# ml4ai/iqlpref

Measured on AMD Instinct MI355X. Metric: iql_grad_steps_per_sec, higher is better.
Workload: dtype bf16; 1 GPU; IQL antmaze-medium-diverse-v2 shapes (S=29 A=8 H=256), 1M-transition device replay, batch 256, one seed per GPU; batch=256, buffer_rows=1000000, graph_unroll=0, graph_launches_per_block=0, eager_steps_per_block=1390

## Files before the change

### iqlpref_amd/csrc/api.hip

```cpp
#include <hip/hip_runtime.h>

#include <algorithm>
#include <cmath>
#include <cstdarg>
#include <cstdio>
#include <cstdlib>
#include <cstring>
#include <new>
#include <vector>

#include "../../include/iqlhip.h"
#include "common.h"
#include "errors.h"
#include "host_plan.h"
#include "iql_deep.h"
#include "iql_step.h"
#include "launchers.h"
#include "step_math.h"

using namespace iqlhip;

static thread_local char g_err[512] = "";
int iqlhip::fail(int code, const char *fmt, ...) {
  va_list ap;
// ... 482 lines not shown
      N.toff_w[k] = N.has_target ? N.off_w[k] : -1;
      N.toff_b[k] = N.has_target ? N.off_b[k] : -1;
    }
  }
  for (int n = 0; n < NT; ++n) {
    const TrainNet &N = D.net[n];
    std::vector<UpdItem> half[2];
    auto put = [&](int layer, int o0, int i0) {
      UpdItem it;
      memset(&it, 0, sizeof(it));
      it.net = n, it.layer = layer, it.o0 = o0, it.i0 = i0;
      it.Odim = (layer == 2) ? N.out_dim : H;
      it.Idim = (layer == 0) ? N.in_dim : H;
      it.Opad = (layer == 2) ? N.out_pad : H;
      it.Kw = (layer == 0) ? N.k1pad : H;
      it.has_target = N.has_target;
      it.group = n == D.net_v ? 1 : (n == D.net_a ? 2 : 0);
      it.off_w = N.off_w[layer], it.off_b = N.off_b[layer], it.toff_w = N.toff_w[layer], it.toff_b = N.toff_b[layer];
      half[(layer == 2 && it.Opad <= 64) ? ((i0 / 32) & 1) : (o0 >= it.Opad / 2 ? 1 : 0)].push_back(it);
    };
    for (int o0 = 0; o0 < H; o0 += 64)
      for (int i0 = 0; i0 < H; i0 += 32) put(1, o0, i0);
    for (int o0 = 0; o0 < H; o0 += strip_rows()) put(0, o0, 0);
    for (int o0 = 0; o0 < N.out_pad; o0 += 64)
      for (int i0 = 0; i0 < H; i0 += 32) put(2, o0, i0);
    u->n_half0[n] = (int)half[0].size();
    u->net_items[n] = half[0];
    u->net_items[n].insert(u->net_items[n].end(), half[1].begin(), half[1].end());
  }
  std::vector<UpdItem> items;
  {
    std::vector<UpdItem> per_xcd[8];
    deal_items(u, 0, 1, per_xcd);
    items = flatten_table(per_xcd, 0, nullptr, (size_t)(B + 15) / 16);
  }
  auto blocks = [&](WorkspacePlan p) {
    for (int n = 0; n < NT; ++n) {
      TrainNet &N = D.net[n];
      N.wc[0] = p.take<char>((size_t)H * N.k1pad * es);
      N.wc[1] = p.take<char>((size_t)H * H * es);
      N.wc[2] = p.take<char>((size_t)N.out_pad * H * es);
      if (N.has_target) {
        N.tc[0] = p.take<char>((size_t)H * N.k1pad * es);
        N.tc[1] = p.take<char>((size_t)H * H * es);
        N.tc[2] = p.take<char>((size_t)N.out_pad * H * es);
      }
      N.w2ct = p.take<char>((size_t)H * H * es);
      N.w3t = p.take<char>((size_t)H * N.out_pad * es);
    }
    D.xT = p.take<char>((size_t)2 * D.xrows * D.BP * es);
    D.rd = p.take<float>((size_t)B * 2);
    D.actf = p.take<float>((size_t)B * A);
    D.hT = p.take<char>((size_t)NT * 2 * H * D.BP * es);
    D.dz1T = p.take<char>((size_t)NT * H * D.BP * es);
    D.dz2T = p.take<char>((size_t)NT * H * D.BP * es);
    D.dz3T = p.take<char>((size_t)NT * D.opmax * D.BP * es);
    D.outs = p.take<float>((size_t)layer2_parts(H) * B * D.OUTW);
    D.lossp = p.take<float>((size_t)NT * (B / 16));
    D.lsp = p.take<float>((size_t)(B / 16) * A);
    D.ls_snap = p.take<float>((size_t)A);
    t->batch_rows = p.take<float>((size_t)B * stride);
    D.stage_rows = p.take<float>((size_t)B * stride);
    u->own.args = p.take<DevArgs>(1);
    u->own.ctr = p.take<DevCtr>(1);
    u->own.desc = p.take<TrainerDesc>(1);
    u->own.items = p.take<UpdItem>(items.size());
    return p.end();
  };
  const size_t total = blocks(WorkspacePlan());
  if (hipMalloc(&u->ws, total) != hipSuccess)
    return fail(IQLHIP_ERR_NOMEM, "hipMalloc of %zu workspace bytes failed", total);
  if (hipMemset(u->ws, 0, total) != hipSuccess) return fail(IQLHIP_ERR_HIP, "hipMemset failed");
  blocks(WorkspacePlan(u->ws));
  u->own.n_items = (int)items.size();
  u->cur = u->own;

  for (int n = 0; n < NT; ++n)
    for (auto &it : u->net_items[n]) item_pointers(it, D, es);
  for (auto &it : items) item_pointers(it, D, es);
  if (hipMemcpy(u->own.items, items.data(), items.size() * sizeof(UpdItem), hipMemcpyHostToDevice) != hipSuccess)
    return fail(IQLHIP_ERR_HIP, "hipMemcpy of the work items failed");

  const std::vector<EvalSpec> order = eval_order(sh, D.next_off);
  for (int f = 0; f < (int)order.size(); ++f) {
    const auto [net, target, in_off, out_col, slot] = order[f];
    FwdNet &F = D.fwd[f];
    const TrainNet &N = D.net[net];
    F.w1c = target ? N.tc[0] : N.wc[0];
    F.w2c = target ? N.tc[1] : N.wc[1];
    F.w3c = target ? N.tc[2] : N.wc[2];
    const float *base = target ? ar->target : ar->params;
    F.b1 = base + N.off_b[0], F.b2 = base + N.off_b[1], F.b3 = base + N.off_b[2];
    F.in_off = in_off, F.in_dim = N.in_dim, F.k1pad = N.k1pad;
// ... 694 lines not shown
```

### iqlpref_amd/csrc/common.h

```cpp
#pragma once
#include <hip/hip_runtime.h>
#include <stdint.h>

namespace iqlhip {

typedef __attribute__((ext_vector_type(4))) float f32x4;
typedef __attribute__((ext_vector_type(8))) __bf16 bf16x8;

constexpr int WAVE = 64;

__device__ __forceinline__ uint16_t f2bf(float x) {
  return __builtin_bit_cast(uint16_t, (__bf16)x);
}
__device__ __forceinline__ float bf2f(uint16_t h) {
  return __builtin_bit_cast(float, (uint32_t)h << 16);
}
__device__ __forceinline__ float rbf(float x) { return bf2f(f2bf(x)); }

#define IQL_AS1 __attribute__((address_space(1)))
template <class T>
__device__ __forceinline__ T ldg(const T *p) {
  return *(const T IQL_AS1 *)p;
}
template <class T>
// ... 100 lines not shown
  return v;
}

__host__ __device__ inline int round_up(int x, int m) { return (x + m - 1) / m * m; }

template <class P>
__host__ __device__ inline size_t fidx(int f, int k, int nk) {
  return ((((size_t)(f >> 4) * nk + k / P::KM) * 64) + ((k % P::KM) / P::EPV) * 16 + (f & 15)) * P::EPV +
         (k % P::EPV);
}
template <class P>
__host__ __device__ inline size_t frag_off(int ft, int ks, int nk, int lane) {
  return (((size_t)ft * nk + ks) * 64 + lane) * P::EPV;
}

struct Philox4 {
  uint32_t x, y, z, w;
};
__device__ __forceinline__ Philox4 philox4x32_10(uint32_t c0, uint32_t c1, uint32_t c2,
                                                 uint32_t c3, uint32_t k0, uint32_t k1) {
#pragma unroll
  for (int i = 0; i < 10; ++i) {
    const uint32_t hi0 = __umulhi(0xD2511F53u, c0), lo0 = 0xD2511F53u * c0;
    const uint32_t hi1 = __umulhi(0xCD9E8D57u, c2), lo1 = 0xCD9E8D57u * c2;
    c0 = hi1 ^ c1 ^ k0;
    c1 = lo1;
    c2 = hi0 ^ c3 ^ k1;
    c3 = lo0;
    k0 += 0x9E3779B9u;
    k1 += 0xBB67AE85u;
  }
  return Philox4{c0, c1, c2, c3};
}
constexpr uint32_t STREAM_INDEX = 0, STREAM_DROPOUT1 = 1, STREAM_DROPOUT2 = 2, STREAM_MLP_DROPOUT = 3;

__device__ __forceinline__ int64_t philox_index(uint64_t seed, uint64_t step, uint32_t row,
                                                uint64_t n_rows) {
  const Philox4 r = philox4x32_10(row, (uint32_t)step, (uint32_t)(step >> 32), STREAM_INDEX,
                                  (uint32_t)seed, (uint32_t)(seed >> 32));
  return (int64_t)((uint64_t)r.x % n_rows);
}

}
```

### iqlpref_amd/csrc/iql_step.h

```cpp
#pragma once
#include <hip/hip_runtime.h>
#include <stdint.h>

namespace iqlhip {

constexpr int MAX_CRITICS = 8;
constexpr int MAX_TRAIN = MAX_CRITICS + 2;
constexpr int MAX_FWD = 2 * MAX_CRITICS + 3;

struct FwdNet {
  const void *w1c, *w2c, *w3c;
  const float *b1, *b2, *b3;
  int32_t in_off;
  int32_t in_dim, k1pad;
  int32_t out_dim, out_pad;
  int32_t out_col;
  int32_t train_slot;
  int32_t tanh_out;
  int32_t dropout;
  int32_t stage;
};

struct TrainNet {
  int64_t off_w[3], off_b[3];
// ... 4 lines not shown
  void *tc[3];
  int32_t in_dim, k1pad, out_dim, out_pad;
  int32_t has_target;
};

struct TrainerDesc {
  int32_t S, A, H, B, BP, OUTW, k1max;
  int32_t E, ntrain, nfwd, net_v, net_a;
  int32_t out_v, out_qt, out_nv, out_mean;
  int32_t stage_stride, next_off;
  int32_t opmax, xrows;
  int32_t deterministic, has_dropout;
  int32_t prefetch;
  int32_t polyak_convex;
  float two_over_B, inv_E;
  float discount, tau, beta, iql_tau;
  float one_m_tau;
  float drop_scale;
  uint32_t drop_thr;
  int32_t NB;
  uint64_t seed;
  float *stage_rows;
  void *xT;
  float *rd;
  float *actf;
  void *hT;
  void *dz1T;
  void *dz2T;
  void *dz3T;
  float *outs;
  float *lossp;
  float *lsp;
  float *ls_snap;
  float *params, *exp_avg, *exp_avg_sq, *target, *grads;
  int64_t off_log_std;
  unsigned long long *dbg;
  double beta1, beta2, eps;
  int64_t t_max;
  FwdNet fwd[MAX_FWD];
  TrainNet net[MAX_TRAIN];
};

struct DevArgs {
  const float *rows;
  int64_t n_rows;
  int32_t row_stride;
  int32_t idx_mode;
  const int64_t *idx;
  const uint8_t *drop_keep;
  float *losses_out;
  int64_t base_step;
  double lr_q, lr_v, lr_a_base;
  int64_t n_steps;
  uint64_t generation;
  const int32_t *n_valid;
};

struct AdamCoef {
  float one_m_b1, b2, one_m_b2, neg_step[3], bc2_sqrt, eps;
  float inv_bc2_sqrt, pad_;
};

struct DevCtr {
  int64_t ctr[2];
  int64_t coef_step;
  AdamCoef coef;
// ... 36 lines not shown
```

### iqlpref_amd/csrc/iql_step.hip

```cpp
#include <algorithm>

#include "common.h"
#include "host_plan.h"
#include "iql_step.h"
#include "step_math.h"

namespace iqlhip {

constexpr int SLAB = 16;

#ifdef IQL_STAMPS
#define STAMP(kern, slot)                                                                   \
  do {                                                                                      \
    if (D.dbg && threadIdx.x == 0 && blockIdx.x < 512) {                                                      \
      unsigned long long *d_ = D.dbg + (((size_t)(kern) * 512 + blockIdx.x) * 8 + (slot)) * 2; \
      d_[0] = wall_clock64();                                                               \
      d_[1] = clock64();                                                                    \
    }                                                                                       \
  } while (0)
#else
#define STAMP(kern, slot) \
  do {                    \
  } while (0)
#endif
// ... 96 lines not shown
  return make_uint2(pk_bf16(t0, t1), pk_bf16(t2, t3));
}

template <bool BF16>
__device__ __forceinline__ void load4T(const typename Prec<BF16>::T *src, float v[4]) {
  if constexpr (BF16) {
    const uint2 u = ldg8(src);
    v[0] = bf2f((uint16_t)(u.x & 0xffff));
    v[1] = bf2f((uint16_t)(u.x >> 16));
    v[2] = bf2f((uint16_t)(u.y & 0xffff));
    v[3] = bf2f((uint16_t)(u.y >> 16));
  } else {
    const float4 f = __builtin_bit_cast(float4, ldg16(src));
    v[0] = f.x, v[1] = f.y, v[2] = f.z, v[3] = f.w;
  }
}

__device__ __forceinline__ void dropout_keep4(const TrainerDesc &D, const DevArgs &A, int64_t step,
                                              int layer, int rowblk, int col, bool keep[4]) {
  if (A.drop_keep) {
    const uint8_t *m = A.drop_keep +
                       (((size_t)(step - A.base_step) * 2 + layer) * D.B + (size_t)rowblk * 4) * D.H + col;
#pragma unroll
    for (int i = 0; i < 4; ++i) keep[i] = ldg(m + (size_t)i * D.H) != 0;
  } else {
    const Philox4 ph = philox4x32_10((uint32_t)(rowblk * D.H + col), (uint32_t)step,
                                     (uint32_t)((uint64_t)step >> 32),
                                     layer == 0 ? STREAM_DROPOUT1 : STREAM_DROPOUT2,
                                     (uint32_t)D.seed, (uint32_t)(D.seed >> 32));
    keep[0] = ph.x >= D.drop_thr;
    keep[1] = ph.y >= D.drop_thr;
    keep[2] = ph.z >= D.drop_thr;
    keep[3] = ph.w >= D.drop_thr;
  }
}

template <bool BF16, int H, class Issue, class Fill>
__device__ __forceinline__ void mlp_slab(const FwdNet &N, const TrainerDesc &D, const DevArgs *Ap,
                                         int64_t step, int slab, char *smem, float *out, int out_stride,
                                         int64_t row0, int64_t n_valid, Issue issue, Fill fill) {
  using K = KCfg<BF16, H>;
  using P = Prec<BF16>;
  using T = typename P::T;
  const int tid = threadIdx.x, lane = tid & 63;
  const int wave = __builtin_amdgcn_readfirstlane(tid >> 6);
  const int r = lane & 15, q = lane >> 4;
  constexpr int HP = K::HP, TPW = K::TPW;
  const int K1P = D.k1max + P::EPV;
  T *xs = reinterpret_cast<T *>(smem);
  T *h1 = xs + SLAB * K1P;
  T *h2 = h1 + SLAB * HP;
  float *red = reinterpret_cast<float *>(h2 + SLAB * HP);

  STAMP(0, 0);
  pin_s(D.hT), pin_s(D.BP), pin_s(N.train_slot), pin_s(N.dropout), pin_s(N.b3), pin_s(N.out_dim);
  pin_s(N.out_col), pin_s(N.tanh_out), pin_s(N.out_pad), pin_s(out), pin_s(out_stride), pin_s(n_valid);
  issue();
  const int nk1 = N.k1pad / P::KM;
  const int nt3 = N.out_pad / 16;
  float bias1[TPW], bias2[TPW];
#pragma unroll
  for (int jj = 0; jj < TPW; ++jj) {
    bias1[jj] = ldg(N.b1 + 16 * (wave * TPW + jj) + r);
    bias2[jj] = ldg(N.b2 + 16 * (wave * TPW + jj) + r);
  }
  float bias3[2];
// ... 124 lines not shown
__device__ __forceinline__ void stage_rows16(const TrainerDesc &D, const DevArgs &A, int64_t step, int row0,
                                             int row_step, int tid) {
  using P = Prec<BF16>;
  using T = typename P::T;
  const int rr = tid >> 4, l16 = tid & 15;
  const int B = D.B, nq = D.stage_stride >> 2, S = D.S, SA = D.S + D.A, nkb = D.BP / P::KM;
  T *const xT = reinterpret_cast<T *>(D.xT) + (size_t)(step & 1) * D.xrows * D.BP;
  for (int row = row0 + rr; row < B; row += row_step) {
    int64_t ix;
    if (A.idx_mode == 1)
      ix = ldg(A.idx + (size_t)(step - A.base_step) * B + row);
    else if (A.idx_mode == 2)
      ix = row;
    else
      ix = philox_index(D.seed, (uint64_t)step, (uint32_t)row, (uint64_t)A.n_rows);
    ix = ix < 0 ? 0 : (ix >= A.n_rows ? A.n_rows - 1 : ix);
    const float *src = A.rows + (size_t)ix * A.row_stride;
    float *dst = D.stage_rows + (size_t)row * D.stage_stride;
    for (int c = l16; c < nq; c += 16) {
      const float4 v4 = __builtin_bit_cast(float4, ldg16(src + 4 * c));
      stg16(dst + 4 * c, v4);
      const float v[4] = {v4.x, v4.y, v4.z, v4.w};
#pragma unroll
      for (int e = 0; e < 4; ++e) {
        const int col = 4 * c + e;
        if (col < SA) stg(xT + fidx<P>(col, row, nkb), P::from_f32(v[e]));
        if (col >= S && col < SA) stg(D.actf + (size_t)row * D.A + (col - S), v[e]);
        if (col >= SA && col < SA + 2) stg(D.rd + (size_t)row * 2 + (col - SA), v[e]);
      }
    }
  }
}

template <bool BF16>
__global__ __launch_bounds__(256) void k_stage(const TrainerDesc *__restrict__ Dp,
                                               const DevArgs *__restrict__ Ap,
                                               const DevCtr *__restrict__ Cp) {
  Dp += blockIdx.y, Ap += blockIdx.y, Cp += blockIdx.y;
  stage_rows16<BF16>(*Dp, *Ap, Cp->ctr[0], blockIdx.x * 16, gridDim.x * 16, threadIdx.x);
}

__global__ __launch_bounds__(256) void k_pad_rows(const uint2 *__restrict__ src, uint2 *__restrict__ dst, int64_t n,
                                                  int rows, int rows_padded, int w8) {
  const int64_t total = n * rows_padded * w8;
  for (int64_t e = (int64_t)blockIdx.x * 256 + threadIdx.x; e < total; e += (int64_t)gridDim.x * 256) {
    const int64_t row = e / w8, blk = row / rows_padded;
    const int w = (int)(e - row * w8), r = (int)(row - blk * rows_padded);
    dst[e] = src[(blk * rows + (r < rows ? r : 0)) * w8 + w];
  }
}

__device__ __forceinline__ void write_adam_coef(const TrainerDesc &D, const DevArgs &A, int64_t t1,
                                                AdamCoef *out);

template <bool BF16, int H>
struct FCfg {
  using P = Prec<BF16>;
  static constexpr int TPW = H / 64;
  static constexpr int SPL = TPW >= 4 ? 4 : TPW;
  static constexpr int HQ = H / SPL;
  static constexpr int NK2 = H / P::KM;
  static constexpr int NK3 = HQ / P::KM;
  static constexpr int NK1 = BF16 ? 4 : 8;
  static constexpr int HP = H + P::EPV;
  static constexpr int HQP = HQ + P::EPV;
  static_assert(HQ == 64, "one 16-column tile per wave and part");
};

template <bool BF16, int H, int MT, int PW>
__global__ __launch_bounds__(256, 3) void k_forward(const TrainerDesc *__restrict__ Dp,
                                                 const DevArgs *__restrict__ Ap,
                                                 const DevCtr *__restrict__ Cp, const int nsl_,
                                                 const int nfwd_) {
  using C = FCfg<BF16, H>;
  using P = Prec<BF16>;
  using T = typename P::T;
  constexpr int ROWS = 16 * MT, TPW = C::TPW, SPL = C::SPL, HP = C::HP, HQP = C::HQP;
  constexpr int NPG = SPL / PW;
  static_assert(SPL % PW == 0 && PW <= 2, "parts per work-group: 1 or 2, dividing the parts");
  Dp += blockIdx.y, Ap += blockIdx.y, Cp += blockIdx.y;
  const TrainerDesc &D = *Dp;
  const int idx_ = blockIdx.x >> 3;
  const int per_job = nsl_ * NPG;
  const int fnet = (idx_ / per_job) * 8 + (blockIdx.x & 7);
  const int rest = idx_ % per_job;
  const int slab = rest / NPG;
  const int part0 = __builtin_amdgcn_readfirstlane((rest % NPG) * PW);
  if (fnet > nfwd_) return;
  if (fnet == nfwd_) {
    if (rest == 0 && threadIdx.x == 0) {
      STAMP(0, 0);
      write_adam_coef(D, *Ap, Cp->ctr[0] + 1, const_cast<AdamCoef *>(&Cp->coef));
      const_cast<DevCtr *>(Cp)->coef_step = Cp->ctr[0] + 1;
      STAMP(0, 5);
    }
    if (rest == 0 && !D.deterministic && (int)threadIdx.x < D.A)
      stg(D.ls_snap + threadIdx.x, ldg(D.params + D.off_log_std + threadIdx.x));
    return;
  }
  const FwdNet N = D.fwd[fnet];
  const int B = D.B, BP = D.BP, OUTW = D.OUTW, k1max = D.k1max;
  const float *const stage = D.stage_rows;
  const unsigned sstride = (unsigned)D.stage_stride;
  float *const g_outs = D.outs;
  void *const g_hT = D.hT;
  const int64_t step = Cp->ctr[0];
  extern __shared__ __attribute__((aligned(16))) char smem[];
  const int tid = threadIdx.x, lane = tid & 63;
  const int wave = __builtin_amdgcn_readfirstlane(tid >> 6);
  const int r = lane & 15, q = lane >> 4;
  const int K1P = k1max + P::EPV;
  T *xs = reinterpret_cast<T *>(smem);
  T *h1 = xs + ROWS * K1P;
  T *h2 = h1 + ROWS * HP;
  STAMP(0, 0);

  const int rr = tid >> 4, l16 = tid & 15;
  const int lim4 = round_up(N.in_dim, 4) - 4;
  float4 xq[MT][2];
#pragma unroll
  for (int m = 0; m < MT; ++m) {
    const int row_ = slab * ROWS + 16 * m + rr;
    const unsigned row = (unsigned)(row_ < B ? row_ : B - 1);
    const float *src = stage + N.in_off;
#pragma unroll
    for (int j = 0; j < 2; ++j) {
      const int c = 4 * l16 + 64 * j;
      xq[m][j] = __builtin_bit_cast(float4, ldg16(src + (row * sstride + (unsigned)(c < lim4 ? c : lim4))));
    }
  }
  const int nk1 = N.k1pad / P::KM;
  const int nt3 = N.out_pad / 16;
  const int tile2 = part0 * 4 + wave;
  float bias1[TPW], bias3[2];
  {
    const float *b1w = N.b1 + 16 * (wave * TPW);
#pragma unroll
    for (int jj = 0; jj < TPW; ++jj) bias1[jj] = ldg(b1w + 16 * jj + r);
  }
  float bias2[PW];
#pragma unroll
  for (int j = 0; j < PW; ++j) bias2[j] = ldg(N.b2 + 16 * (tile2 + 4 * j) + r);
#pragma unroll
  for (int jt = 0; jt < 2; ++jt)
    bias3[jt] = ldg(N.b3 + (16 * jt + r < N.out_dim ? 16 * jt + r : N.out_dim - 1));
  uint4 w1[C::NK1][TPW], w2[PW][C::NK2], w3[PW][C::NK3][2];
  auto load_w2 = [&]() {
#pragma unroll
    for (int j = 0; j < PW; ++j) {
      const T *W2w = reinterpret_cast<const T *>(N.w2c) + (size_t)(tile2 + 4 * j) * C::NK2 * 64 * P::EPV;
#pragma unroll
      for (int ks = 0; ks < C::NK2; ++ks) w2[j][ks] = ldg16(W2w + ks * 64 * P::EPV + lane * P::EPV);
    }
  };
  auto load_w3 = [&]() {
#pragma unroll
    for (int j = 0; j < PW; ++j) {
      const T *W3w = reinterpret_cast<const T *>(N.w3c) + (size_t)((part0 + j) * C::NK3) * 64 * P::EPV;
#pragma unroll
      for (int ks = 0; ks < C::NK3; ++ks)
#pragma unroll
        for (int jt = 0; jt < 2; ++jt)
          if (jt < nt3) w3[j][ks][jt] = ldg16(W3w + (size_t)(jt * C::NK2 + ks) * 64 * P::EPV + lane * P::EPV);
    }
  };
  {
    const T *W1w = reinterpret_cast<const T *>(N.w1c) + (size_t)(wave * TPW) * nk1 * 64 * P::EPV;
#pragma unroll
    for (int ks = 0; ks < C::NK1; ++ks) {
      if (ks < nk1) {
#pragma unroll
        for (int jj = 0; jj < TPW; ++jj)
          w1[ks][jj] = ldg16(W1w + (size_t)(jj * nk1 + ks) * 64 * P::EPV + lane * P::EPV);
      }
    }
  }
  STAMP(0, 1);

#pragma unroll
  for (int m = 0; m < MT; ++m) {
#pragma unroll
    for (int j = 0; j < 2; ++j) {
      const int c = 4 * l16 + 64 * j;
      const float v[4] = {xq[m][j].x, xq[m][j].y, xq[m][j].z, xq[m][j].w};
      if (c < N.k1pad) {
        T tv[4];
#pragma unroll
        for (int e = 0; e < 4; ++e) tv[e] = P::from_f32(c + e < N.in_dim ? v[e] : 0.f);
        if constexpr (BF16) {
          uint2 u;
          u.x = (uint32_t)tv[0] | ((uint32_t)tv[1] << 16), u.y = (uint32_t)tv[2] | ((uint32_t)tv[3] << 16);
          *reinterpret_cast<uint2 *>(xs + (16 * m + rr) * K1P + c) = u;
        } else {
          *reinterpret_cast<float4 *>(xs + (16 * m + rr) * K1P + c) = make_float4(tv[0], tv[1], tv[2], tv[3]);
        }
      }
    }
  }
  __syncthreads();
  STAMP(0, 2);

  {
    f32x4 acc[MT][TPW];
#pragma unroll
    for (int m = 0; m < MT; ++m)
#pragma unroll
      for (int jj = 0; jj < TPW; ++jj) acc[m][jj] = f32x4{0.f, 0.f, 0.f, 0.f};
#pragma unroll
    for (int ks = 0; ks < C::NK1; ++ks) {
      if (ks < nk1) {
#pragma unroll
        for (int m = 0; m < MT; ++m) {
          const uint4 a = *reinterpret_cast<const uint4 *>(xs + (16 * m + r) * K1P + ks * P::KM + P::EPV * q);
#pragma unroll
          for (int jj = 0; jj < TPW; ++jj) P::mma(a, w1[ks][jj], acc[m][jj]);
        }
      }
    }
    __builtin_amdgcn_sched_barrier(0);
    load_w2();
    __builtin_amdgcn_sched_barrier(0);
    bool lean = false;
    if constexpr (BF16) lean = !N.dropout;
#pragma unroll
    for (int jj = 0; jj < TPW; ++jj) {
      const int tile = wave * TPW + jj;
      const int col = 16 * tile + r;
      const float bias = P::round(bias1[jj]);
      const bool mine = N.train_slot >= 0 && ((tile * SPL) / (4 * TPW)) / PW * PW == part0;
      if (lean) {
        if constexpr (BF16) {
          uint2 u[MT];
#pragma unroll
          for (int m = 0; m < MT; ++m) {
            u[m] = relu_bias_bf16x4(acc[m][jj], bias);
            T *hrow = h1 + (16 * m + 4 * q) * HP + col;
            hrow[0] = (T)(u[m].x & 0xffff), hrow[HP] = (T)(u[m].x >> 16);
            hrow[2 * HP] = (T)(u[m].y & 0xffff), hrow[3 * HP] = (T)(u[m].y >> 16);
          }
          T *plane = reinterpret_cast<T *>(g_hT) + (size_t)(N.train_slot * 2 + 0) * H * BP;
          if constexpr (MT == 2) {
            if (mine && slab * ROWS + ROWS <= B) {
#pragma unroll
              for (int m = 0; m < MT; m += 2) act_store16_pair(plane, col, slab * ROWS + 16 * m, q, BP / P::KM, u[m], u[m + 1]);
            }
          } else {
#pragma unroll
            for (int m = 0; m < MT; ++m)
              if (mine && slab * ROWS + 16 * m < B) act_store8_fwd(plane, fidx<P>(col, slab * ROWS + 16 * m + 4 * q, BP / P::KM), u[m]);
          }
        }
        continue;
      }
#pragma unroll
      for (int m = 0; m < MT; ++m) {
        const int row0 = slab * ROWS + 16 * m;
        float v[4];
#pragma unroll
        for (int i = 0; i < 4; ++i) v[i] = fmaxf(P::round(acc[m][jj][i] + bias), 0.f);
        if (N.dropout) {
          bool keep[4];
          dropout_keep4(D, *Ap, step, 0, (row0 >> 2) + q, col, keep);
#pragma unroll
          for (int i = 0; i < 4; ++i) v[i] = keep[i] ? P::round(v[i] * D.drop_scale) : 0.f;
        }
#pragma unroll
        for (int i = 0; i < 4; ++i) h1[(16 * m + 4 * q + i) * HP + col] = P::from_f32(v[i]);
        if (mine && row0 < B)
          store4T<BF16>(reinterpret_cast<T *>(g_hT) + (size_t)(N.train_slot * 2 + 0) * H * BP +
                            fidx<P>(col, row0 + 4 * q, BP / P::KM), v);
      }
    }
  }
  __syncthreads();
  STAMP(0, 3);

  {
    f32x4 acc[PW][MT];
#pragma unroll
    for (int j = 0; j < PW; ++j)
#pragma unroll
      for (int m = 0; m < MT; ++m) acc[j][m] = f32x4{0.f, 0.f, 0.f, 0.f};
#pragma unroll
    for (int ks = 0; ks < C::NK2; ++ks) {
#pragma unroll
      for (int m = 0; m < MT; ++m) {
        const uint4 a = *reinterpret_cast<const uint4 *>(h1 + (16 * m + r) * HP + ks * P::KM + P::EPV * q);
#pragma unroll
        for (int j = 0; j < PW; ++j) P::mma(a, w2[j][ks], acc[j][m]);
      }
    }
    __builtin_amdgcn_sched_barrier(0);
    load_w3();
    __builtin_amdgcn_sched_barrier(0);
    bool lean = false;
    if constexpr (BF16) lean = !N.dropout;
#pragma unroll
    for (int j = 0; j < PW; ++j) {
      const int col = 16 * (tile2 + 4 * j) + r;
      const float bias = P::round(bias2[j]);
      T *h2j = h2 + j * ROWS * HQP;
      if (lean) {
        if constexpr (BF16) {
          uint2 u[MT];
#pragma unroll
          for (int m = 0; m < MT; ++m) {
            u[m] = relu_bias_bf16x4(acc[j][m], bias);
            T *hrow = h2j + (16 * m + 4 * q) * HQP + 16 * wave + r;
            hrow[0] = (T)(u[m].x & 0xffff), hrow[HQP] = (T)(u[m].x >> 16);
            hrow[2 * HQP] = (T)(u[m].y & 0xffff), hrow[3 * HQP] = (T)(u[m].y >> 16);
          }
          T *plane = reinterpret_cast<T *>(g_hT) + (size_t)(N.train_slot * 2 + 1) * H * BP;
          if constexpr (MT == 2) {
            if (N.train_slot >= 0 && slab * ROWS + ROWS <= B) {
#pragma unroll
              for (int m = 0; m < MT; m += 2) act_store16_pair(plane, col, slab * ROWS + 16 * m, q, BP / P::KM, u[m], u[m + 1]);
            }
          } else {
#pragma unroll
            for (int m = 0; m < MT; ++m)
              if (N.train_slot >= 0 && slab * ROWS + 16 * m < B)
                act_store8_fwd(plane, fidx<P>(col, slab * ROWS + 16 * m + 4 * q, BP / P::KM), u[m]);
          }
        }
        continue;
      }
#pragma unroll
      for (int m = 0; m < MT; ++m) {
        const int row0 = slab * ROWS + 16 * m;
        float v[4];
#pragma unroll
        for (int i = 0; i < 4; ++i) v[i] = fmaxf(P::round(acc[j][m][i] + bias), 0.f);
        if (N.dropout) {
          bool keep[4];
          dropout_keep4(D, *Ap, step, 1, (row0 >> 2) + q, col, keep);
#pragma unroll
          for (int i = 0; i < 4; ++i) v[i] = keep[i] ? P::round(v[i] * D.drop_scale) : 0.f;
        }
#pragma unroll
        for (int i = 0; i < 4; ++i) h2j[(16 * m + 4 * q + i) * HQP + 16 * wave + r] = P::from_f32(v[i]);
        if (N.train_slot >= 0 && row0 < B)
          store4T<BF16>(reinterpret_cast<T *>(g_hT) + (size_t)(N.train_slot * 2 + 1) * H * BP +
                            fidx<P>(col, row0 + 4 * q, BP / P::KM), v);
      }
    }
  }
  __syncthreads();
  STAMP(0, 4);

  for (int pr = wave; pr < MT * PW; pr += 4) {
    const int m = pr % MT, j = pr / MT;
    const T *h2j = h2 + j * ROWS * HQP;
    f32x4 acc3[2] = {f32x4{0.f, 0.f, 0.f, 0.f}, f32x4{0.f, 0.f, 0.f, 0.f}};
#pragma unroll
    for (int ks = 0; ks < C::NK3; ++ks) {
      const uint4 a = *reinterpret_cast<const uint4 *>(h2j + (16 * m + r) * HQP + ks * P::KM + P::EPV * q);
#pragma unroll
      for (int jt = 0; jt < 2; ++jt) {
        if (jt < nt3) {
          if constexpr (PW == 1) {
            P::mma(a, w3[0][ks][jt], acc3[jt]);
          } else {
            if (j == 0) P::mma(a, w3[0][ks][jt], acc3[jt]);
            else P::mma(a, w3[PW - 1][ks][jt], acc3[jt]);
          }
        }
      }
    }
    float *outp = g_outs + (size_t)(part0 + j) * B * OUTW;
    const int row0 = slab * ROWS + 16 * m + 4 * q;
// ... 15 lines not shown
                                                        const DevArgs *__restrict__ Ap,
                                                        const DevCtr *__restrict__ Cp, const int nsl_,
                                                        const int nfwd_) {
  using C = FCfg<true, H>;
  using P = Prec<true>;
  using T = typename P::T;
  constexpr int ROWS = 64, MT = ROWS / 16, NW = 8;
  constexpr int TPW = H / (16 * NW);
  constexpr int SPL = C::SPL, HP = C::HP, NK2 = C::NK2, NK3 = C::NK3;
  static_assert(H == 256 && TPW == 2 && SPL == 4, "k_forward_tp is built for H = 256");
  Dp += blockIdx.y, Ap += blockIdx.y, Cp += blockIdx.y;
  const TrainerDesc &D = *Dp;
  const int idx_ = blockIdx.x >> 3;
  const int fnet = (idx_ / nsl_) * 8 + (blockIdx.x & 7);
  const int slab = idx_ % nsl_;
  if (fnet > nfwd_) return;
  if (fnet == nfwd_) {
    if (slab == 0 && threadIdx.x == 0) {
      STAMP(0, 0);
      write_adam_coef(D, *Ap, Cp->ctr[0] + 1, const_cast<AdamCoef *>(&Cp->coef));
      const_cast<DevCtr *>(Cp)->coef_step = Cp->ctr[0] + 1;
      STAMP(0, 5);
    }
    if (slab == 0 && !D.deterministic && (int)threadIdx.x < D.A)
      stg(D.ls_snap + threadIdx.x, ldg(D.params + D.off_log_std + threadIdx.x));
    return;
  }
  const FwdNet N = D.fwd[fnet];
  const int B = D.B, BP = D.BP, OUTW = D.OUTW, k1max = D.k1max;
  const float *const stage = D.stage_rows;
  const unsigned sstride = (unsigned)D.stage_stride;
  float *const g_outs = D.outs;
  void *const g_hT = D.hT;
  const int64_t step = Cp->ctr[0];
  extern __shared__ __attribute__((aligned(16))) char smem[];
  const int tid = threadIdx.x, lane = tid & 63;
  const int wave = __builtin_amdgcn_readfirstlane(tid >> 6);
  const int r = lane & 15, q = lane >> 4;
  const int K1P = k1max + P::EPV;
  T *xs = reinterpret_cast<T *>(smem);
  T *h1 = xs + ROWS * K1P;
  T *h2 = h1 + ROWS * HP;
  STAMP(0, 0);

  const int rr = tid >> 3, l8 = tid & 7;
  const int lim4 = round_up(N.in_dim, 4) - 4;
  float4 xq[4];
  {
    const int row_ = slab * ROWS + rr;
    const unsigned row = (unsigned)(row_ < B ? row_ : B - 1);
    const float *src = stage + N.in_off;
#pragma unroll
    for (int j = 0; j < 4; ++j) {
      const int c = 4 * l8 + 32 * j;
      xq[j] = __builtin_bit_cast(float4, ldg16(src + (row * sstride + (unsigned)(c < lim4 ? c : lim4))));
    }
  }
  const int nk1 = N.k1pad / P::KM;
  const int nt3 = N.out_pad / 16;
  const int tile0 = wave * TPW;
  const int part = tile0 / 4;
  float bias1[TPW], bias2[TPW], bias3[2];
#pragma unroll
  for (int jj = 0; jj < TPW; ++jj) {
    bias1[jj] = ldg(N.b1 + 16 * (tile0 + jj) + r);
    bias2[jj] = ldg(N.b2 + 16 * (tile0 + jj) + r);
  }
#pragma unroll
  for (int jt = 0; jt < 2; ++jt)
    bias3[jt] = ldg(N.b3 + (16 * jt + r < N.out_dim ? 16 * jt + r : N.out_dim - 1));
  uint4 w1[C::NK1][TPW], w2[TPW][NK2], w3[NK3][2];
  {
    const T *W1w = reinterpret_cast<const T *>(N.w1c) + (size_t)tile0 * nk1 * 64 * P::EPV;
#pragma unroll
    for (int ks = 0; ks < C::NK1; ++ks) {
      if (ks < nk1) {
#pragma unroll
        for (int jj = 0; jj < TPW; ++jj)
          w1[ks][jj] = ldg16(W1w + (size_t)(jj * nk1 + ks) * 64 * P::EPV + lane * P::EPV);
      }
    }
  }
  auto load_w23 = [&]() {
#pragma unroll
    for (int jj = 0; jj < TPW; ++jj) {
      const T *W2w = reinterpret_cast<const T *>(N.w2c) + (size_t)(tile0 + jj) * NK2 * 64 * P::EPV;
#pragma unroll
      for (int ks = 0; ks < NK2; ++ks) w2[jj][ks] = ldg16(W2w + ks * 64 * P::EPV + lane * P::EPV);
    }
    const T *W3w = reinterpret_cast<const T *>(N.w3c) + (size_t)(part * NK3) * 64 * P::EPV;
#pragma unroll
    for (int ks = 0; ks < NK3; ++ks)
#pragma unroll
      for (int jt = 0; jt < 2; ++jt)
        if (jt < nt3) w3[ks][jt] = ldg16(W3w + (size_t)(jt * NK2 + ks) * 64 * P::EPV + lane * P::EPV);
  };
  load_w23();
  STAMP(0, 1);

#pragma unroll
  for (int j = 0; j < 4; ++j) {
    const int c = 4 * l8 + 32 * j;
    const float v[4] = {xq[j].x, xq[j].y, xq[j].z, xq[j].w};
    if (c < N.k1pad) {
      T tv[4];
#pragma unroll
      for (int e = 0; e < 4; ++e) tv[e] = P::from_f32(c + e < N.in_dim ? v[e] : 0.f);
      uint2 u;
      u.x = (uint32_t)tv[0] | ((uint32_t)tv[1] << 16), u.y = (uint32_t)tv[2] | ((uint32_t)tv[3] << 16);
      *reinterpret_cast<uint2 *>(xs + rr * K1P + c) = u;
    }
  }
  __syncthreads();
  STAMP(0, 2);

  const bool store_h = N.train_slot >= 0;
  {
    f32x4 acc[MT][TPW];
#pragma unroll
    for (int m = 0; m < MT; ++m)
#pragma unroll
      for (int jj = 0; jj < TPW; ++jj) acc[m][jj] = f32x4{0.f, 0.f, 0.f, 0.f};
#pragma unroll
    for (int ks = 0; ks < C::NK1; ++ks) {
      if (ks < nk1) {
#pragma unroll
        for (int m = 0; m < MT; ++m) {
          const uint4 a = *reinterpret_cast<const uint4 *>(xs + (16 * m + r) * K1P + ks * P::KM + P::EPV * q);
#pragma unroll
          for (int jj = 0; jj < TPW; ++jj) P::mma(a, w1[ks][jj], acc[m][jj]);
        }
      }
    }
    STAMP(0, 6);
#pragma unroll
    for (int jj = 0; jj < TPW; ++jj) {
      const int col = 16 * (tile0 + jj) + r;
      const float bias = P::round(bias1[jj]);
      if constexpr (!DROP) {
        uint2 u[MT];
#pragma unroll
        for (int m = 0; m < MT; ++m) {
          u[m] = relu_bias_bf16x4(acc[m][jj], bias);
          T *hrow = h1 + (16 * m + 4 * q) * HP + col;
          hrow[0] = (T)(u[m].x & 0xffff), hrow[HP] = (T)(u[m].x >> 16);
          hrow[2 * HP] = (T)(u[m].y & 0xffff), hrow[3 * HP] = (T)(u[m].y >> 16);
        }
        if (store_h) {
          T *plane = reinterpret_cast<T *>(g_hT) + (size_t)(N.train_slot * 2 + 0) * H * BP;
#pragma unroll
          for (int m = 0; m < MT; m += 2)
            act_store16_pair(plane, col, slab * ROWS + 16 * m, q, BP / P::KM, u[m], u[m + 1]);
        }
        continue;
      }
#pragma unroll
      for (int m = 0; m < MT; ++m) {
        const int row0 = slab * ROWS + 16 * m;
        float v[4];
#pragma unroll
        for (int i = 0; i < 4; ++i) v[i] = fmaxf(P::round(acc[m][jj][i] + bias), 0.f);
        if (N.dropout) {
          bool keep[4];
          dropout_keep4(D, *Ap, step, 0, (row0 >> 2) + q, col, keep);
#pragma unroll
          for (int i = 0; i < 4; ++i) v[i] = keep[i] ? P::round(v[i] * D.drop_scale) : 0.f;
        }
#pragma unroll
        for (int i = 0; i < 4; ++i) h1[(16 * m + 4 * q + i) * HP + col] = P::from_f32(v[i]);
        if (store_h)
          store4T<true>(reinterpret_cast<T *>(g_hT) + (size_t)(N.train_slot * 2 + 0) * H * BP +
                            fidx<P>(col, row0 + 4 * q, BP / P::KM), v);
      }
    }
  }
  __syncthreads();
  STAMP(0, 3);

  {
    f32x4 acc[TPW][MT];
#pragma unroll
    for (int jj = 0; jj < TPW; ++jj)
#pragma unroll
      for (int m = 0; m < MT; ++m) acc[jj][m] = f32x4{0.f, 0.f, 0.f, 0.f};
#pragma unroll
    for (int ks = 0; ks < NK2; ++ks) {
#pragma unroll
      for (int m = 0; m < MT; ++m) {
        const uint4 a = *reinterpret_cast<const uint4 *>(h1 + (16 * m + r) * HP + ks * P::KM + P::EPV * q);
#pragma unroll
        for (int jj = 0; jj < TPW; ++jj) P::mma(a, w2[jj][ks], acc[jj][m]);
      }
    }
    STAMP(0, 7);
#pragma unroll
    for (int jj = 0; jj < TPW; ++jj) {
      const int col = 16 * (tile0 + jj) + r;
      const float bias = P::round(bias2[jj]);
      if constexpr (!DROP) {
        uint2 u[MT];
#pragma unroll
        for (int m = 0; m < MT; ++m) {
          u[m] = relu_bias_bf16x4(acc[jj][m], bias);
          T *hrow = h2 + (16 * m + 4 * q) * HP + col;
          hrow[0] = (T)(u[m].x & 0xffff), hrow[HP] = (T)(u[m].x >> 16);
          hrow[2 * HP] = (T)(u[m].y & 0xffff), hrow[3 * HP] = (T)(u[m].y >> 16);
        }
        if (store_h) {
          T *plane = reinterpret_cast<T *>(g_hT) + (size_t)(N.train_slot * 2 + 1) * H * BP;
#pragma unroll
          for (int m = 0; m < MT; m += 2)
            act_store16_pair(plane, col, slab * ROWS + 16 * m, q, BP / P::KM, u[m], u[m + 1]);
        }
        continue;
      }
#pragma unroll
      for (int m = 0; m < MT; ++m) {
        const int row0 = slab * ROWS + 16 * m;
        float v[4];
#pragma unroll
        for (int i = 0; i < 4; ++i) v[i] = fmaxf(P::round(acc[jj][m][i] + bias), 0.f);
        if (N.dropout) {
          bool keep[4];
          dropout_keep4(D, *Ap, step, 1, (row0 >> 2) + q, col, keep);
#pragma unroll
          for (int i = 0; i < 4; ++i) v[i] = keep[i] ? P::round(v[i] * D.drop_scale) : 0.f;
        }
#pragma unroll
        for (int i = 0; i < 4; ++i) h2[(16 * m + 4 * q + i) * HP + col] = P::from_f32(v[i]);
        if (store_h)
          store4T<true>(reinterpret_cast<T *>(g_hT) + (size_t)(N.train_slot * 2 + 1) * H * BP +
                            fidx<P>(col, row0 + 4 * q, BP / P::KM), v);
      }
    }
  }
  __syncthreads();
  STAMP(0, 4);

  {
    float *outp = g_outs + (size_t)part * B * OUTW;
#pragma unroll
    for (int mm = 0; mm < MT / 2; ++mm) {
      const int m = (wave & 1) * (MT / 2) + mm;
      f32x4 acc3[2] = {f32x4{0.f, 0.f, 0.f, 0.f}, f32x4{0.f, 0.f, 0.f, 0.f}};
#pragma unroll
      for (int ks = 0; ks < NK3; ++ks) {
        const uint4 a = *reinterpret_cast<const uint4 *>(h2 + (16 * m + r) * HP + 64 * part + ks * P::KM + P::EPV * q);
#pragma unroll
        for (int jt = 0; jt < 2; ++jt)
          if (jt < nt3) P::mma(a, w3[ks][jt], acc3[jt]);
      }
      const int row0 = slab * ROWS + 16 * m + 4 * q;
#pragma unroll
      for (int jt = 0; jt < 2; ++jt) {
        const int col = 16 * jt + r;
        if (jt < nt3 && col < N.out_dim) {
          const float bias = part == 0 ? P::round(bias3[jt]) : 0.f;
// ... 685 lines not shown
      float p = ls;
      adam_apply<BF16>(p, pm, pv, g, coef, coef.neg_step[2]);
      stg(D.params + o, p), stg(D.exp_avg + o, pm), stg(D.exp_avg_sq + o, pv);
      if (D.grads) stg(D.grads + o, g);
    }
    if (tid >= 64 && tid < 64 + nt) {
      const int n = tid - 64;
      float s = 0.f;
      for (int k = 0; k < nslab; ++k) s += sred[n * nslab + k];
      int nv = B;
      if constexpr (!BF16 || CNT) nv = VALID_ROWS(A.n_valid, A, t1 - 1, D.NB);
      sred[nl + na + n] = s / (float)nv;
    }
    __syncthreads();
    if (tid == 64) {
      const float vl = sred[nl + na + D.net_v];
      float ql = 0.f;
      for (int e = 0; e < D.E; ++e) ql += sred[nl + na + e];
      ql = ql / (float)D.E;
      const float al = sred[nl + na + D.net_a];
      Cp->last_losses[0] = vl, Cp->last_losses[1] = ql, Cp->last_losses[2] = al;
      Cp->loss_sum[0] += vl, Cp->loss_sum[1] += ql, Cp->loss_sum[2] += al;
      if (A.losses_out) {
        float *lo = A.losses_out + (size_t)(t1 - 1 - A.base_step) * 3;
        stg(lo, vl), stg(lo + 1, ql), stg(lo + 2, al);
      }
      Cp->ctr[0] = t1;
    }
    STAMP(2, 4);
    return;
  }

  if (it.net < 0) {
    if (D.prefetch && (A.idx_mode == 0 || (A.idx_mode == 1 && t1 - A.base_step < A.n_steps)))
      stage_rows16<BF16>(D, A, t1, it.o0 * (UT / 16), it.i0 * (UT / 16), tid);
    return;
  }
  const int L = it.layer;
  const int Odim = it.Odim, Idim = it.Idim, Kw = it.Kw, Opad = it.Opad;
  const int Ipad = round_up(Idim, 16);
  const int o0 = it.o0, i0 = it.i0;
  const float neg_step =
      it.group == 0 ? coef.neg_step[0] : (it.group == 1 ? coef.neg_step[1] : coef.neg_step[2]);
  const bool has_target = it.has_target != 0;
  const int nk = BP / P::KM;
  const int kh = (BF16 && nk >= 16) ? (nk / (2 * UKC)) * UKC : nk;
  const bool ksplit = kh < nk;
  pin_s(D.tau), pin_s(D.one_m_tau), pin_s(D.polyak_convex);
  pin_s(it.off_w), pin_s(it.toff_w), pin_s(it.off_b), pin_s(it.toff_b), pin_s(it.wc), pin_s(it.tc);
  pin_s(it.w2ct), pin_s(it.Xsrc), pin_s(it.Zsrc), pin_s(Kw), pin_s(neg_step);
  pin_s(coef.one_m_b1), pin_s(coef.b2), pin_s(coef.one_m_b2), pin_s(coef.bc2_sqrt), pin_s(coef.eps);
  pin_s(coef.inv_bc2_sqrt);

  if (L == 0) {
    const int TLD = Ipad + 4;
    const int64_t fbase = it.off_w + (int64_t)o0 * Idim, tbase = it.toff_w + (int64_t)o0 * Idim;
    constexpr int UNE = LAT ? (USR * UMAXI + UT - 1) / UT : 1;
    constexpr int UN4 = LAT ? 1 : (USR * UMAXI / 4 + UT - 1) / UT;
    const int n_el = USR * Idim, n4 = n_el >> 2;
    float pf[UNE], mf[UNE], vf[UNE], tf[UNE];
    float4 pf4[UN4], mf4[UN4], vf4[UN4], tf4[UN4];
    float pb, mb, vb, tb;
    auto load_state = [&]() {
      if constexpr (LAT) {
#pragma unroll
        for (int k = 0; k < UNE; ++k) {
          const int e = tid + UT * k;
          const int ec = e < n_el ? e : n_el - 1;
// ... 548 lines not shown
  const int64_t fwd_wgs = (int64_t)D.nfwd * (D.B / 64) * n_seeds, bwd_wgs = (int64_t)D.ntrain * (D.B / 32) * n_seeds;
  const bool fwd_tp = fwd_wgs >= 72 && fwd_wgs <= 256;
  return backward ? (fwd_tp && bwd_wgs >= 144 && bwd_wgs <= 256) : fwd_tp;
}
hipError_t prepare_step_kernels() {
  hipError_t e = hipFuncSetAttribute(reinterpret_cast<const void *>(k_forward_tp<256, false>),
                                     hipFuncAttributeMaxDynamicSharedMemorySize, 160 * 1024);
  if (e != hipSuccess) return e;
  return hipFuncSetAttribute(reinterpret_cast<const void *>(k_forward_tp<256, true>),
                             hipFuncAttributeMaxDynamicSharedMemorySize, 160 * 1024);
}
static size_t fwd_tp_smem_bytes(int H, int k1max) { return (size_t)64 * ((k1max + 8) + 2 * (H + 8)) * 2; }

hipError_t launch_forward(bool bf16, const TrainerDesc &D, const TrainerDesc *dD, const DevArgs *a,
                          const DevCtr *c, int n_seeds, hipStream_t st) {
  if (use_tp(bf16, D, n_seeds, false)) {
    const int nsl64 = D.B / 64;
    const int grid = 8 * ((D.nfwd + 1 + 7) / 8) * nsl64;
    if (D.has_dropout)
      hipLaunchKernelGGL((k_forward_tp<256, true>), dim3(grid, n_seeds), dim3(512), fwd_tp_smem_bytes(256, D.k1max), st,
                         dD, a, c, nsl64, D.nfwd);
    else
      hipLaunchKernelGGL((k_forward_tp<256, false>), dim3(grid, n_seeds), dim3(512), fwd_tp_smem_bytes(256, D.k1max), st,
                         dD, a, c, nsl64, D.nfwd);
    return hipGetLastError();
  }
  const int mt = fwd_row_tiles(D.B, n_seeds), nsl = (D.B + 16 * mt - 1) / (16 * mt);
  const int pw = fwd_parts_per_wg(D.B, D.H, n_seeds);
  const int grid = 8 * ((D.nfwd + 1 + 7) / 8) * nsl * (layer2_parts(D.H) / pw);
  const size_t sm = fwd_smem_bytes(bf16, D.H, D.k1max, mt, pw);
  dispatch_h(bf16, D.H, [&](auto BF, auto HH) {
    auto go = [&](auto PW) {
      with_const<2, 1>(mt, [&](auto MT) {
        hipLaunchKernelGGL((k_forward<CV(BF), CV(HH), CV(MT), CV(PW)>), dim3(grid, n_seeds), dim3(256), sm, st, dD, a,
                           c, nsl, D.nfwd);
      });
    };
    if constexpr (CV(HH) >= 128) {
      if (pw == 2) return go(Int<2>{});
    }
    go(Int<1>{});
  });
  return hipGetLastError();
}
static int bwd_parts_per_wg(int B, int H, int n_seeds) {
  return ((int64_t)B * n_seeds >= 512 && layer2_parts(H) % 2 == 0) ? 2 : 1;
}
hipError_t launch_backward(bool bf16, const TrainerDesc &D, const TrainerDesc *dD, const DevArgs *a,
                           DevCtr *c, int n_seeds, hipStream_t st, bool counts) {
  if (use_tp(bf16, D, n_seeds, true)) {
    const int nslab32 = D.B / 32;
    const int nxn = (D.ntrain <= 4 && nslab32 % 2 == 0) ? 2 : 1;
    const int grid = 8 * ((D.ntrain * nxn + 7) / 8) * (nslab32 / nxn);
    hipLaunchKernelGGL((k_backward_tp<256>), dim3(grid, n_seeds), dim3(512), 2 * bwd_smem_bytes(true, 256), st, dD, a, c,
                       nslab32, D.ntrain, nxn);
    return hipGetLastError();
  }
  const int pw = bwd_parts_per_wg(D.B, D.H, n_seeds);
  const int grid = 8 * ((layer2_parts(D.H) / pw * D.ntrain + 7) / 8) * (D.B / SLAB);
  const size_t sm = bwd_smem_bytes(bf16, D.H);
  const bool pre = (int64_t)D.B * n_seeds < 1024;
  dispatch_h(bf16, D.H, [&](auto BF, auto HH) {
    with_const<true, false>(counts, [&](auto NV) {
      auto go = [&](auto PRE, auto PW) {
        hipLaunchKernelGGL((k_backward<CV(BF), CV(HH), CV(PRE), CV(PW), CV(NV)>), dim3(grid, n_seeds), dim3(256), sm,
                           st, dD, a, c, D.B / SLAB, D.ntrain);
      };
      if constexpr (CV(HH) >= 128) {
// ... 69 lines not shown
```

Measured before the change: 66410 steps/s.

## Precompute dropout keep masks in staging pass instead of inline Philox in forward

Moves the Philox dropout mask generation out of the forward kernels and into the row-staging pass of the previous step (and k_stage), writing packed 4-bit keep masks to a new workspace buffer. The forward kernels then load these bytes up front, pack them into registers, and skip the per-element Philox work. A DROP template flag also compiles dropout out entirely when the trainer has no dropout. This trades RNG compute on the forward critical path for extra global memory traffic, plus more items in the update table when dropout is on.

Measured after the change: 67330 steps/s, median of 6. +1.4%, better.

```diff
diff --git a/iqlpref_amd/csrc/api.hip b/iqlpref_amd/csrc/api.hip
--- a/iqlpref_amd/csrc/api.hip
+++ b/iqlpref_amd/csrc/api.hip
@@ -538,7 +538,8 @@
   {
     std::vector<UpdItem> per_xcd[8];
     deal_items(u, 0, 1, per_xcd);
-    items = flatten_table(per_xcd, 0, nullptr, (size_t)(B + 15) / 16);
+    const size_t rows16 = (size_t)(B + 15) / 16;
+    items = flatten_table(per_xcd, 0, nullptr, D.has_dropout && rows16 < 32 ? 32 : rows16);
   }
   auto blocks = [&](WorkspacePlan p) {
     for (int n = 0; n < NT; ++n) {
@@ -565,6 +566,7 @@
     D.lossp = p.take<float>((size_t)NT * (B / 16));
     D.lsp = p.take<float>((size_t)(B / 16) * A);
     D.ls_snap = p.take<float>((size_t)A);
+    D.keepb = D.has_dropout ? p.take<uint8_t>((size_t)2 * (B / 4) * H) : nullptr;
     t->batch_rows = p.take<float>((size_t)B * stride);
     D.stage_rows = p.take<float>((size_t)B * stride);
     u->own.args = p.take<DevArgs>(1);
diff --git a/iqlpref_amd/csrc/common.h b/iqlpref_amd/csrc/common.h
--- a/iqlpref_amd/csrc/common.h
+++ b/iqlpref_amd/csrc/common.h
@@ -156,6 +156,20 @@
   }
   return Philox4{c0, c1, c2, c3};
 }
+__device__ __forceinline__ Philox4 philox4x32_10_wide(uint32_t c0, uint32_t c1, uint32_t c2,
+                                                      uint32_t c3, uint32_t k0, uint32_t k1) {
+#pragma unroll
+  for (int i = 0; i < 10; ++i) {
+    const uint64_t p0 = (uint64_t)0xD2511F53u * c0, p1 = (uint64_t)0xCD9E8D57u * c2;
+    c0 = (uint32_t)(p1 >> 32) ^ c1 ^ k0;
+    c1 = (uint32_t)p1;
+    c2 = (uint32_t)(p0 >> 32) ^ c3 ^ k1;
+    c3 = (uint32_t)p0;
+    k0 += 0x9E3779B9u;
+    k1 += 0xBB67AE85u;
+  }
+  return Philox4{c0, c1, c2, c3};
+}
 constexpr uint32_t STREAM_INDEX = 0, STREAM_DROPOUT1 = 1, STREAM_DROPOUT2 = 2, STREAM_MLP_DROPOUT = 3;
 
 __device__ __forceinline__ int64_t philox_index(uint64_t seed, uint64_t step, uint32_t row,
diff --git a/iqlpref_amd/csrc/iql_step.h b/iqlpref_amd/csrc/iql_step.h
--- a/iqlpref_amd/csrc/iql_step.h
+++ b/iqlpref_amd/csrc/iql_step.h
@@ -60,6 +60,7 @@
   float *lossp;
   float *lsp;
   float *ls_snap;
+  uint8_t *keepb;
   float *params, *exp_avg, *exp_avg_sq, *target, *grads;
   int64_t off_log_std;
   unsigned long long *dbg;
diff --git a/iqlpref_amd/csrc/iql_step.hip b/iqlpref_amd/csrc/iql_step.hip
--- a/iqlpref_amd/csrc/iql_step.hip
+++ b/iqlpref_amd/csrc/iql_step.hip
@@ -152,6 +152,19 @@
     keep[1] = ph.y >= D.drop_thr;
     keep[2] = ph.z >= D.drop_thr;
     keep[3] = ph.w >= D.drop_thr;
+  }
+}
+
+__device__ __forceinline__ void keep4_fwd(const TrainerDesc &D, const DevArgs &A, const uint8_t *inj,
+                                          const DevCtr *Cp, uint32_t kb, int layer, int rowblk, int col,
+                                          bool keep[4]) {
+  if (inj) {
+    const uint8_t *m = inj + (((size_t)(Cp->ctr[0] - A.base_step) * 2 + layer) * D.B + (size_t)rowblk * 4) * D.H + col;
+#pragma unroll
+    for (int i = 0; i < 4; ++i) keep[i] = ldg(m + (size_t)i * D.H) != 0;
+  } else {
+#pragma unroll
+    for (int i = 0; i < 4; ++i) keep[i] = ((kb >> i) & 1u) != 0;
   }
 }
 
@@ -342,12 +355,30 @@
   }
 }
 
+__device__ __forceinline__ void draw_keep_plane(const TrainerDesc &D, const DevArgs &A, int64_t step, int part,
+                                                int nparts, int tid, int nthr) {
+  if (!D.has_dropout || A.drop_keep) return;
+  const int per_layer = (D.B >> 2) * D.H;
+  const uint32_t thr = D.drop_thr;
+  for (int e = part * nthr + tid; e < 2 * per_layer; e += nparts * nthr) {
+    const int layer = e >= per_layer ? 1 : 0;
+    const Philox4 ph = philox4x32_10_wide((uint32_t)(e - layer * per_layer), (uint32_t)step,
+                                          (uint32_t)((uint64_t)step >> 32),
+                                          layer == 0 ? STREAM_DROPOUT1 : STREAM_DROPOUT2,
+                                          (uint32_t)D.seed, (uint32_t)(D.seed >> 32));
+    const uint32_t bits = (ph.x >= thr ? 1u : 0u) | (ph.y >= thr ? 2u : 0u) | (ph.z >= thr ? 4u : 0u) |
+                          (ph.w >= thr ? 8u : 0u);
+    stg(D.keepb + e, (uint8_t)bits);
+  }
+}
+
 template <bool BF16>
 __global__ __launch_bounds__(256) void k_stage(const TrainerDesc *__restrict__ Dp,
                                                const DevArgs *__restrict__ Ap,
                                                const DevCtr *__restrict__ Cp) {
   Dp += blockIdx.y, Ap += blockIdx.y, Cp += blockIdx.y;
   stage_rows16<BF16>(*Dp, *Ap, Cp->ctr[0], blockIdx.x * 16, gridDim.x * 16, threadIdx.x);
+  draw_keep_plane(*Dp, *Ap, Cp->ctr[0], blockIdx.x, gridDim.x, threadIdx.x, 256);
 }
 
 __global__ __launch_bounds__(256) void k_pad_rows(const uint2 *__restrict__ src, uint2 *__restrict__ dst, int64_t n,
@@ -377,7 +408,7 @@
   static_assert(HQ == 64, "one 16-column tile per wave and part");
 };
 
-template <bool BF16, int H, int MT, int PW>
+template <bool BF16, int H, int MT, int PW, bool DROP>
 __global__ __launch_bounds__(256, 3) void k_forward(const TrainerDesc *__restrict__ Dp,
                                                  const DevArgs *__restrict__ Ap,
                                                  const DevCtr *__restrict__ Cp, const int nsl_,
@@ -414,7 +445,9 @@
   const unsigned sstride = (unsigned)D.stage_stride;
   float *const g_outs = D.outs;
   void *const g_hT = D.hT;
-  const int64_t step = Cp->ctr[0];
+  const uint8_t *const keepb = DROP ? D.keepb : nullptr;
+  const uint8_t *const inj = DROP ? Ap->drop_keep : nullptr;
+  if constexpr (DROP) pin_s(inj), pin_s(D.drop_scale);
   extern __shared__ __attribute__((aligned(16))) char smem[];
   const int tid = threadIdx.x, lane = tid & 63;
   const int wave = __builtin_amdgcn_readfirstlane(tid >> 6);
@@ -451,6 +484,18 @@
   float bias2[PW];
 #pragma unroll
   for (int j = 0; j < PW; ++j) bias2[j] = ldg(N.b2 + 16 * (tile2 + 4 * j) + r);
+  uint32_t kb1[MT][TPW] = {}, kb2[PW][MT] = {};
+  if constexpr (DROP) {
+#pragma unroll
+    for (int m = 0; m < MT; ++m) {
+      const int rb_ = ((slab * ROWS + 16 * m) >> 2) + q;
+      const uint8_t *kr = keepb + (size_t)(rb_ < (B >> 2) ? rb_ : (B >> 2) - 1) * H + r;
+#pragma unroll
+      for (int jj = 0; jj < TPW; ++jj) kb1[m][jj] = ldg(kr + 16 * (wave * TPW + jj));
+#pragma unroll
+      for (int j = 0; j < PW; ++j) kb2[j][m] = ldg(kr + (size_t)(B >> 2) * H + 16 * (tile2 + 4 * j));
+    }
+  }
 #pragma unroll
   for (int jt = 0; jt < 2; ++jt)
     bias3[jt] = ldg(N.b3 + (16 * jt + r < N.out_dim ? 16 * jt + r : N.out_dim - 1));
@@ -507,6 +552,17 @@
       }
     }
   }
+  uint32_t kp1 = 0, kp2 = 0;
+  if constexpr (DROP) {
+#pragma unroll
+    for (int m = 0; m < MT; ++m) {
+#pragma unroll
+      for (int jj = 0; jj < TPW; ++jj) kp1 |= kb1[m][jj] << (4 * (m * TPW + jj));
+#pragma unroll
+      for (int j = 0; j < PW; ++j) kp2 |= kb2[j][m] << (4 * (j * MT + m));
+    }
+    asm volatile("" : "+v"(kp1), "+v"(kp2));
+  }
   __syncthreads();
   STAMP(0, 2);
 
@@ -530,8 +586,7 @@
     __builtin_amdgcn_sched_barrier(0);
     load_w2();
     __builtin_amdgcn_sched_barrier(0);
-    bool lean = false;
-    if constexpr (BF16) lean = !N.dropout;
+    const bool lean = BF16 && (!DROP || !N.dropout);
 #pragma unroll
     for (int jj = 0; jj < TPW; ++jj) {
       const int tile = wave * TPW + jj;
@@ -568,11 +623,13 @@
         float v[4];
 #pragma unroll
         for (int i = 0; i < 4; ++i) v[i] = fmaxf(P::round(acc[m][jj][i] + bias), 0.f);
-        if (N.dropout) {
-          bool keep[4];
-          dropout_keep4(D, *Ap, step, 0, (row0 >> 2) + q, col, keep);
-#pragma unroll
-          for (int i = 0; i < 4; ++i) v[i] = keep[i] ? P::round(v[i] * D.drop_scale) : 0.f;
+        if constexpr (DROP) {
+          if (N.dropout) {
+            bool keep[4];
+            keep4_fwd(D, *Ap, inj, Cp, kp1 >> (4 * (m * TPW + jj)), 0, (row0 >> 2) + q, col, keep);
+#pragma unroll
+            for (int i = 0; i < 4; ++i) v[i] = keep[i] ? P::round(v[i] * D.drop_scale) : 0.f;
+          }
         }
 #pragma unroll
         for (int i = 0; i < 4; ++i) h1[(16 * m + 4 * q + i) * HP + col] = P::from_f32(v[i]);
@@ -603,8 +660,7 @@
     __builtin_amdgcn_sched_barrier(0);
     load_w3();
     __builtin_amdgcn_sched_barrier(0);
-    bool lean = false;
-    if constexpr (BF16) lean = !N.dropout;
+    const bool lean = BF16 && (!DROP || !N.dropout);
 #pragma unroll
     for (int j = 0; j < PW; ++j) {
       const int col = 16 * (tile2 + 4 * j) + r;
@@ -641,11 +697,13 @@
         float v[4];
 #pragma unroll
         for (int i = 0; i < 4; ++i) v[i] = fmaxf(P::round(acc[j][m][i] + bias), 0.f);
-        if (N.dropout) {
-          bool keep[4];
-          dropout_keep4(D, *Ap, step, 1, (row0 >> 2) + q, col, keep);
-#pragma unroll
-          for (int i = 0; i < 4; ++i) v[i] = keep[i] ? P::round(v[i] * D.drop_scale) : 0.f;
+        if constexpr (DROP) {
+          if (N.dropout) {
+            bool keep[4];
+            keep4_fwd(D, *Ap, inj, Cp, kp2 >> (4 * (j * MT + m)), 1, (row0 >> 2) + q, col, keep);
+#pragma unroll
+            for (int i = 0; i < 4; ++i) v[i] = keep[i] ? P::round(v[i] * D.drop_scale) : 0.f;
+          }
         }
 #pragma unroll
         for (int i = 0; i < 4; ++i) h2j[(16 * m + 4 * q + i) * HQP + 16 * wave + r] = P::from_f32(v[i]);
@@ -727,7 +785,9 @@
   const unsigned sstride = (unsigned)D.stage_stride;
   float *const g_outs = D.outs;
   void *const g_hT = D.hT;
-  const int64_t step = Cp->ctr[0];
+  const uint8_t *const keepb = DROP ? D.keepb : nullptr;
+  const uint8_t *const inj = DROP ? Ap->drop_keep : nullptr;
+  if constexpr (DROP) pin_s(inj), pin_s(D.drop_scale);
   extern __shared__ __attribute__((aligned(16))) char smem[];
   const int tid = threadIdx.x, lane = tid & 63;
   const int wave = __builtin_amdgcn_readfirstlane(tid >> 6);
@@ -764,6 +824,18 @@
 #pragma unroll
   for (int jt = 0; jt < 2; ++jt)
     bias3[jt] = ldg(N.b3 + (16 * jt + r < N.out_dim ? 16 * jt + r : N.out_dim - 1));
+  uint32_t kb1[MT][TPW] = {}, kb2[TPW][MT] = {};
+  if constexpr (DROP) {
+#pragma unroll
+    for (int m = 0; m < MT; ++m) {
+      const uint8_t *kr = keepb + (size_t)(((slab * ROWS + 16 * m) >> 2) + q) * H + 16 * tile0 + r;
+#pragma unroll
+      for (int jj = 0; jj < TPW; ++jj) {
+        kb1[m][jj] = ldg(kr + 16 * jj);
+        kb2[jj][m] = ldg(kr + (size_t)(B >> 2) * H + 16 * jj);
+      }
+    }
+  }
   uint4 w1[C::NK1][TPW], w2[TPW][NK2], w3[NK3][2];
   {
     const T *W1w = reinterpret_cast<const T *>(N.w1c) + (size_t)tile0 * nk1 * 64 * P::EPV;
@@ -806,6 +878,15 @@
       *reinterpret_cast<uint2 *>(xs + rr * K1P + c) = u;
     }
   }
+  uint32_t kp1 = 0, kp2 = 0;
+  if constexpr (DROP) {
+#pragma unroll
+    for (int m = 0; m < MT; ++m)
+#pragma unroll
+      for (int jj = 0; jj < TPW; ++jj)
+        kp1 |= kb1[m][jj] << (4 * (m * TPW + jj)), kp2 |= kb2[jj][m] << (4 * (jj * MT + m));
+    asm volatile("" : "+v"(kp1), "+v"(kp2));
+  }
   __syncthreads();
   STAMP(0, 2);
 
@@ -857,7 +938,7 @@
         for (int i = 0; i < 4; ++i) v[i] = fmaxf(P::round(acc[m][jj][i] + bias), 0.f);
         if (N.dropout) {
           bool keep[4];
-          dropout_keep4(D, *Ap, step, 0, (row0 >> 2) + q, col, keep);
+          keep4_fwd(D, *Ap, inj, Cp, kp1 >> (4 * (m * TPW + jj)), 0, (row0 >> 2) + q, col, keep);
 #pragma unroll
           for (int i = 0; i < 4; ++i) v[i] = keep[i] ? P::round(v[i] * D.drop_scale) : 0.f;
         }
@@ -917,7 +998,7 @@
         for (int i = 0; i < 4; ++i) v[i] = fmaxf(P::round(acc[jj][m][i] + bias), 0.f);
         if (N.dropout) {
           bool keep[4];
-          dropout_keep4(D, *Ap, step, 1, (row0 >> 2) + q, col, keep);
+          keep4_fwd(D, *Ap, inj, Cp, kp2 >> (4 * (jj * MT + m)), 1, (row0 >> 2) + q, col, keep);
 #pragma unroll
           for (int i = 0; i < 4; ++i) v[i] = keep[i] ? P::round(v[i] * D.drop_scale) : 0.f;
         }
@@ -1669,8 +1750,13 @@
   }
 
   if (it.net < 0) {
-    if (D.prefetch && (A.idx_mode == 0 || (A.idx_mode == 1 && t1 - A.base_step < A.n_steps)))
+    if (D.prefetch && (A.idx_mode == 0 || (A.idx_mode == 1 && t1 - A.base_step < A.n_steps))) {
       stage_rows16<BF16>(D, A, t1, it.o0 * (UT / 16), it.i0 * (UT / 16), tid);
+      const int ng = (D.B + UT / 16 - 1) / (UT / 16);
+      const int nd = it.i0 > ng ? ng : 0;
+      if (it.o0 >= nd) draw_keep_plane(D, A, t1, it.o0 - nd, it.i0 - nd, tid, UT);
+    }
+    STAMP(2, 4);
     return;
   }
   const int L = it.layer;
@@ -2285,8 +2371,10 @@
   dispatch_h(bf16, D.H, [&](auto BF, auto HH) {
     auto go = [&](auto PW) {
       with_const<2, 1>(mt, [&](auto MT) {
-        hipLaunchKernelGGL((k_forward<CV(BF), CV(HH), CV(MT), CV(PW)>), dim3(grid, n_seeds), dim3(256), sm, st, dD, a,
-                           c, nsl, D.nfwd);
+        with_const<false, true>(D.has_dropout != 0, [&](auto DROP) {
+          hipLaunchKernelGGL((k_forward<CV(BF), CV(HH), CV(MT), CV(PW), CV(DROP)>), dim3(grid, n_seeds), dim3(256), sm,
+                             st, dD, a, c, nsl, D.nfwd);
+        });
       });
     };
     if constexpr (CV(HH) >= 128) {
```
